# xinjuezou-whi/Open_Duck_Playground

Measured on AMD Instinct MI355X. Metric: env steps/sec (all envs) open_duck_mini_v2 flat, 4096 envs, 1/2/4/8 GPUs, higher is better.
Workload: dtype f32; 1 GPU; C2: flat_terrain, no imitation, 4096 envs per GPU, episode_length 1000 + auto-reset; envs_per_gpu=4096, total_envs=4096, substeps=10, parallelism=env-shard x1, step_kernel=throughput

## Files before the change

### open_duck_playground_amd/csrc/duck_lspairs.h

```cpp
#pragma once
#include "duck_math.h"

typedef float f2v __attribute__((ext_vector_type(2)));

DK float ls_flag_select(float x) { return x < 0.0f ? 1.0f : 0.0f; }
DK float ls_flag_sat(float x) { return __builtin_amdgcn_fmed3f(x * -0x1p127f, 0.0f, 1.0f); }
template <bool SAT>
DK float ls_flag(float x) {
  return SAT ? ls_flag_sat(x) : ls_flag_select(x);
}

template <class Md>
constexpr bool ls_pairs() {
#ifdef DUCK_SCALAR_TWINS
  return false;
#else
  return !(Md::FLOOR_TYPE == 1 && Md::NLIM <= 16);
#endif
}
```

### open_duck_playground_amd/csrc/duck_team.h

```cpp
#pragma once
#include <utility>

#include "duck_ldlpairs.h"
#include "duck_lspairs.h"
#include "duck_mcols.h"
#include "duck_physics.h"

constexpr int TEAM = 16;
constexpr int TEAM_WG = 16;
constexpr int TPB = TEAM * TEAM_WG;
typedef __attribute__((address_space(3))) int lds_int;
typedef float f4v __attribute__((ext_vector_type(4)));
typedef __attribute__((address_space(3))) f4v lds_f4;

DK float frcp(float x) { return __builtin_amdgcn_rcpf(x); }
DK float vsel(unsigned long long m, float t, float f) {
  float r;
  asm("v_cndmask_b32_e64 %0, %1, %2, %3" : "=v"(r) : "v"(f), "v"(t), "s"(m));
  return r;
}

DK float imp_of(const float* solimp, float pos) {
  const float dmin = fminf(fmaxf(solimp[0], 0.0001f), 0.9999f), dmax = fminf(fmaxf(solimp[1], 0.0001f), 0.9999f);
  const float width = fmaxf(1e-15f, solimp[2]), mid = fminf(fmaxf(solimp[3], 0.0001f), 0.9999f);
// ... 2293 lines not shown
      for (int q = 0; q < 3; q++) L[FB + 3 * f + q] = -t[q];
    }
    TSYNC();
    auto sep_of = [&](const float* u) {
      float mx1 = -1e30f, mn2 = 1e30f;
#pragma unroll
      for (int k = 0; k < NH; k++) {
        mx1 = fmaxf(mx1, dot3(u, V1[k]));
        mn2 = fminf(mn2, dot3(u, V2[k]));
      }
      return mn2 - mx1;
    };
    constexpr int NONE = 1 << 20;
    constexpr float TIE = Md::HULL_SAT_TIE;
    constexpr int NFL = (2 * NF + TEAM - 1) / TEAM;
    float fs[NFL], fmx = -1e30f, anysep = 0.0f;
#pragma unroll
    for (int k = 0; k < NFL; k++) {
      const int a = lane + TEAM * k;
      fs[k] = -1e30f;
      if (a < 2 * NF) {
        const int o = a < NF ? FA + 3 * a : FB + 3 * (a - NF);
        const float u[3] = {L[o], L[o + 1], L[o + 2]};
        const float sp = sep_of(u);
        anysep += sp > 0.0f ? 1.0f : 0.0f;
        fs[k] = sp;
      }
      fmx = fmaxf(fmx, fs[k]);
    }
    if (tsum(anysep) > 0.0f) return;
    const float ftop = tmaxf(fmx);
    int mine = NONE;
#pragma unroll
    for (int k = NFL - 1; k >= 0; k--)
      if (fs[k] >= ftop - TIE) mine = lane + TEAM * k;
    const int fbest = tmini(mine);
    float myf = fs[0];
#pragma unroll
    for (int k = 1; k < NFL; k++) myf = fbest / TEAM == k ? fs[k] : myf;
    float best = __shfl(myf, fbest % TEAM, TEAM);
    int btype = fbest / NF, bi = fbest - btype * NF, bj = 0;
    float u_best[3];
    {
      const int o = btype == 0 ? FA + 3 * bi : FB + 3 * bi;
      for (int q = 0; q < 3; q++) u_best[q] = L[o + q];
    }
    constexpr int NEL = (NE + TEAM - 1) / TEAM;
    float EBr[NEL][3], Cr[NEL][3], Dr[NEL][3], DxC[NEL][3];
#pragma unroll
    for (int k = 0; k < NEL; k++) {
      const int e2 = lane + TEAM * k, e2c = e2 < NE ? e2 : 0;
      const int fc = HEF[e2c][0], fd = HEF[e2c][1];
      for (int q = 0; q < 3; q++) {
        EBr[k][q] = L[EB + 3 * e2c + q];
        Cr[k][q] = L[FB + 3 * fc + q];
        Dr[k][q] = L[FB + 3 * fd + q];
      }
      cross3(DxC[k], Dr[k], Cr[k]);
    }
    float esep = -1e30f, eu[3] = {0.0f, 0.0f, 1.0f};
    int eidx = NONE;
    for (int e1 = 0; e1 < NE; e1++) {
      const float ea[3] = {L[EA + 3 * e1], L[EA + 3 * e1 + 1], L[EA + 3 * e1 + 2]};
      const int fa = HEF[e1][0], fb = HEF[e1][1];
      const float A[3] = {L[FA + 3 * fa], L[FA + 3 * fa + 1], L[FA + 3 * fa + 2]};
      const float B[3] = {L[FA + 3 * fb], L[FA + 3 * fb + 1], L[FA + 3 * fb + 2]};
      float BxA[3];
      cross3(BxA, B, A);
      float sepq = 0.0f;
#pragma unroll
      for (int k = 0; k < NEL; k++) {
        const int e2 = lane + TEAM * k;
        const float CBA = dot3(Cr[k], BxA), DBA = dot3(Dr[k], BxA), ADC = dot3(A, DxC[k]), BDC = dot3(B, DxC[k]);
        if (e2 < NE && CBA * DBA < 0.0f && ADC * BDC < 0.0f && CBA * BDC > 0.0f) {
          float u[3];
          cross3(u, ea, EBr[k]);
          const float un = sqrtf(dot3(u, u));
          if (!(un < 1e-6f * sqrtf(dot3(ea, ea)) * sqrtf(dot3(EBr[k], EBr[k])))) {
            u[0] /= un; u[1] /= un; u[2] /= un;
            if (dot3(u, cc) < 0.0f) { u[0] = -u[0]; u[1] = -u[1]; u[2] = -u[2]; }
            const float sp = sep_of(u);
            sepq += sp > 0.0f ? 1.0f : 0.0f;
            if (sp > esep) { esep = sp; eidx = e1 * NE + e2; eu[0] = u[0]; eu[1] = u[1]; eu[2] = u[2]; }
          }
        }
      }
      if (tsum(sepq) > 0.0f) return;
    }
    const float em = tmaxf(esep);
    const int ebest = tmini(esep == em ? eidx : NONE);
    float u_edge[3];
    for (int q = 0; q < 3; q++) u_edge[q] = __shfl(eu[q], (ebest % NE) % TEAM, TEAM);
    if (ebest < NONE && em > best + TIE) {
      best = em;
      btype = 2;
      bi = ebest / NE;
      bj = ebest - bi * NE;
      for (int q = 0; q < 3; q++) u_best[q] = u_edge[q];
    }
    TSYNC();
    float fr[9];
    make_frame(fr, u_best);
    if (btype == 2) {
      float a0[3], a1[3], b0[3], b1[3];
      pick3<NH>(V1, HE[bi][0], a0);
      pick3<NH>(V1, HE[bi][1], a1);
      pick3<NH>(V2, HE[bj][0], b0);
      pick3<NH>(V2, HE[bj][1], b1);
      float d1[3], d2[3], r[3];
      for (int a = 0; a < 3; a++) { d1[a] = a1[a] - a0[a]; d2[a] = b1[a] - b0[a]; r[a] = a0[a] - b0[a]; }
      const float A = dot3(d1, d1), E = dot3(d2, d2), F = dot3(d2, r), C = dot3(d1, r), B = dot3(d1, d2);
      const float den = A * E - B * B;
      float sc = den > 1e-15f ? (B * F - C * E) / den : 0.0f;
      sc = fminf(fmaxf(sc, 0.0f), 1.0f);
      float tt = E > 1e-15f ? (B * sc + F) / E : 0.0f;
      if (tt < 0.0f) { tt = 0.0f; sc = A > 1e-15f ? -C / A : 0.0f; }
      else if (tt > 1.0f) { tt = 1.0f; sc = A > 1e-15f ? (B - C) / A : 0.0f; }
      sc = fminf(fmaxf(sc, 0.0f), 1.0f);
      float pos[3];
      for (int a = 0; a < 3; a++) pos[a] = 0.5f * (a0[a] + sc * d1[a] + b0[a] + tt * d2[a]);
      if (lane == 0) Ph::store_contact(L, slot0, best, pos, fr);
      return;
    }
    const bool ref1 = btype == 0;
    const float* Rr = ref1 ? R1 : R2;
    const float* Ri = ref1 ? R2 : R1;
    const float* pr = ref1 ? p1 : p2;
    float fn[3];
    mulmv3(fn, Rr, HN[bi]);
    const float off = Md::hull_face_offset_d()[bi] + dot3(fn, pr);
    int finc = 0;
    float dmin = 1e30f;
    for (int f = 0; f < NF; f++) {
      float ni[3];
      mulmv3(ni, Ri, HN[f]);
      const float dd = dot3(ni, fn);
      finc = dd < dmin ? f : finc;
      dmin = fminf(dmin, dd);
    }
    constexpr int MFV = Md::HULL_MAXFV, CLIPMAX = 2 * MFV;
    constexpr int PA = EA, PB = EA + 3 * CLIPMAX;
    static_assert(PB + 3 * CLIPMAX <= FA, "clip scratch must fit in the edge storage");
    const int(*FV)[MFV] = Md::hull_face_vert_d();
    const int* FNV = Md::hull_face_nv_d();
    auto vtx = [&](bool h1, int k, float* out) {
      float o1[3], o2[3];
      pick3<NH>(V1, k, o1);
      pick3<NH>(V2, k, o2);
      for (int q = 0; q < 3; q++) out[q] = h1 ? o1[q] : o2[q];
    };
    int np = FNV[finc];
    for (int i = 0; i < np; i++) {
      float v[3];
      vtx(!ref1, FV[finc][i], v);
      for (int q = 0; q < 3; q++) L[PA + 3 * i + q] = v[q];
    }
    int src = PA, dst = PB;
    const int nr = FNV[bi];
    for (int i = 0; i < nr && np > 0; i++) {
      float a[3], b[3], ab[3], sd[3];
      vtx(ref1, FV[bi][i], a);
      vtx(ref1, FV[bi][i + 1 < nr ? i + 1 : 0], b);
      for (int q = 0; q < 3; q++) ab[q] = b[q] - a[q];
      cross3(sd, ab, fn);
      int nt = 0;
      for (int j = 0; j < np; j++) {
        const int jn = j + 1 < np ? j + 1 : 0;
        const float P[3] = {L[src + 3 * j], L[src + 3 * j + 1], L[src + 3 * j + 2]};
        const float Q[3] = {L[src + 3 * jn], L[src + 3 * jn + 1], L[src + 3 * jn + 2]};
        const float dp = sd[0] * (P[0] - a[0]) + sd[1] * (P[1] - a[1]) + sd[2] * (P[2] - a[2]);
        const float dq = sd[0] * (Q[0] - a[0]) + sd[1] * (Q[1] - a[1]) + sd[2] * (Q[2] - a[2]);
        if (dp <= 0.0f && nt < CLIPMAX) {
          for (int q = 0; q < 3; q++) L[dst + 3 * nt + q] = P[q];
          nt++;
        }
        if ((dp <= 0.0f) != (dq <= 0.0f) && nt < CLIPMAX) {
          const float tt = dp / (dp - dq);
          for (int q = 0; q < 3; q++) L[dst + 3 * nt + q] = P[q] + tt * (Q[q] - P[q]);
          nt++;
        }
      }
      TSYNC();
      np = nt;
      const int sw = src;
      src = dst;
      dst = sw;
    }
    float poly[CLIPMAX][3], depth[CLIPMAX];
    bool mask[CLIPMAX], any = false;
#pragma unroll
    for (int k = 0; k < CLIPMAX; k++) {
      const bool ok = k < np;
      for (int q = 0; q < 3; q++) poly[k][q] = ok ? L[src + 3 * k + q] : 0.0f;
      depth[k] = off - dot3(fn, poly[k]);
      mask[k] = ok && depth[k] > 0.0f;
      any = any || mask[k];
    }
    if (!any) return;
    int idx[4];
    manifold_points<CLIPMAX>(poly, mask, fn, idx);
    if (lane < 4) {
      const int c = lane;
      bool unique = true;
      for (int e = 0; e < 4; e++) unique = unique && !(e < c && idx[e] == idx[c]);
      const float dist = unique ? -pick1<CLIPMAX>(depth, idx[c]) : 1.0f;
      float v[3], pos[3];
      pick3<CLIPMAX>(poly, idx[c], v);
      for (int a = 0; a < 3; a++) pos[a] = v[a] - 0.5f * dist * fn[a];
      Ph::store_contact(L, slot0 + c, dist, pos, fr);
    }
  }

  static DNI void collide_hulls_rare(LP L, int lane) {
    constexpr int p = Md::FOOT_PAIR < 0 ? 0 : Md::FOOT_PAIR;
    const int s1 = cgeom_slot<Md>(Md::pair_geom1[p]), s2 = cgeom_slot<Md>(Md::pair_geom2[p]);
    float p1[3], R1[9], p2[3], R2[9], t[3], c1[3], c2[3];
    Ph::geom_frame(L, s1, p1, R1);
    Ph::geom_frame(L, s2, p2, R2);
    const float hc[3] = {Md::hull_center[0], Md::hull_center[1], Md::hull_center[2]};
    mulmv3(t, R1, hc);
    for (int a = 0; a < 3; a++) c1[a] = p1[a] + t[a];
    mulmv3(t, R2, hc);
    for (int a = 0; a < 3; a++) c2[a] = p2[a] + t[a];
    const float cc[3] = {c2[0] - c1[0], c2[1] - c1[1], c2[2] - c1[2]};
    collide_hulls_team(L, lane, 4 * p, p1, R1, p2, R2, cc);
  }

  static DK void collision(LP L, int lane, const float* hf, const ColPre& P) {
    STAGE_T0();
    if constexpr (Md::FLOOR_TYPE == 1) collide_hfield(L, lane, hf);
    else collide_planes(L, lane, P);
    STAGE_MARK(ST_COLLISION_FLOOR);
    if (Md::FOOT_PAIR >= 0) {
      constexpr int p = Md::FOOT_PAIR;
      const int s1 = cgeom_slot<Md>(Md::pair_geom1[p]), s2 = cgeom_slot<Md>(Md::pair_geom2[p]);
      float p1[3], R1[9], p2[3], R2[9], t[3];
      Ph::geom_frame(L, s1, p1, R1);
      Ph::geom_frame(L, s2, p2, R2);
      float c1[3], c2[3];
      const float hc[3] = {Md::hull_center[0], Md::hull_center[1], Md::hull_center[2]};
      mulmv3(t, R1, hc);
      for (int a = 0; a < 3; a++) c1[a] = p1[a] + t[a];
      mulmv3(t, R2, hc);
      for (int a = 0; a < 3; a++) c2[a] = p2[a] + t[a];
      const float cc[3] = {c2[0] - c1[0], c2[1] - c1[1], c2[2] - c1[2]};
      if (dot3(cc, cc) > 4.0f * Md::hull_radius * Md::hull_radius || boxes_separated(p1, R1, p2, R2)) {
        if (lane < 4) {
          const float nofr[9] = {0, 0, 1, 0, 1, 0, -1, 0, 0};
          const float zero[3] = {L[Ly::COM], L[Ly::COM + 1], L[Ly::COM + 2]};
          Ph::store_contact(L, 4 * p + lane, 1.0f, zero, nofr);
        }
      } else {
        TSYNC();
        STAGE_COUNT_IF(lane == 0, ST_N_FOOT_SAT, 1ull);
        collide_hulls_rare(L, lane);
      }
    }
    TSYNC();
  }

  static DK void make_rows(LP L, int lane) {
    if (lane < NFRIC) {
      const int r = lane, i = fric_dof(r);
      L[Ly::RD + r] = tf(Md::B_FRIC + 3 * r + 1);
      L[Ly::AREF + r] = -tf(Md::B_FRIC + 3 * r + 2) * L[Ly::QVEL + i];
    }
    team_for<NLIM>(lane, [&](int r) {
      const int o = Md::B_LIM + LIMW * r;
      const int i = lim_dof(r), qa = lim_qadr(r);
      const float q = L[Ly::QPOS + qa];
      const float dlo = q - tf(o + 2), dhi = tf(o + 3) - q;
      const float pos = fminf(dlo, dhi) - tf(o + 4);
      const float sgn = dlo < dhi ? 1.0f : -1.0f;
      const float k = tf(o + 5), b = tf(o + 6);
      const float si[5] = {tf(o + 8), tf(o + 9), tf(o + 10), tf(o + 11), tf(o + 12)};
      const float imp = imp_of(si, pos);
      const float R = fmaxf(tf(o + 7) * (1.0f - imp) * frcp(imp), 1e-15f);
      const bool active = pos < 0.0f;
      L[Ly::RD + R_LIM + r] = active ? frcp(R) : 0.0f;
      L[Ly::AREF + R_LIM + r] = active ? (-b * sgn * L[Ly::QVEL + i] - k * imp * pos) : 0.0f;
      L[Ly::LSGN + r] = sgn;
    });
    if (lane < NCON) {
      const int slot = lane, p = slot >> 2, o = Md::B_PAIR + PAIRW * p;
      float SL[6], SR[6];
      for (int k = 0; k < 6; k++) { SL[k] = L[Ly::CVEL + 6 * Md::LFOOT_BODY + k]; SR[k] = L[Ly::CVEL + 6 * Md::RFOOT_BODY + k]; }
      const float pos = L[Ly::CDIST + slot] - tf(o + 4);
      const bool active = pos < 0.0f;
      const float k = tf(o + 5), b = tf(o + 6);
      const float si[5] = {tf(o + 8), tf(o + 9), tf(o + 10), tf(o + 11), tf(o + 12)};
      const float imp = imp_of(si, pos);
      const float R = fmaxf(tf(o + 3) * (1.0f - imp) * frcp(imp), 1e-15f);
      float vel[4];
      contact_jx(L, p, slot, SL, SR, vel);
      for (int e = 0; e < 4; e++) {
        const int row = R_CON + 4 * slot + e;
        L[Ly::RD + row] = active ? frcp(R) : 0.0f;
        L[Ly::AREF + row] = active ? (-b * vel[e] - k * imp * pos) : 0.0f;
      }
    }
    TSYNC();
  }

  struct JxIn {
    int s1, s2;
    float mu, r[3], fr[9];
  };
  static DK JxIn jx_load(LP L, int p, int slot) {
    const int o = Md::B_PAIR + PAIRW * p;
    JxIn J;
    J.s1 = ti(o); J.s2 = ti(o + 1); J.mu = tf(o + 2);
    for (int k = 0; k < 3; k++) J.r[k] = L[Ly::CR + Ly::CRS * slot + k];
    for (int k = 0; k < 9; k++) J.fr[k] = L[Ly::CFR + Ly::CFS * slot + k];
    return J;
  }
  static DK void contact_jx(LP L, int p, int slot, const float* SL, const float* SR, float* out4) {
    contact_jx(jx_load(L, p, slot), SL, SR, out4);
  }
  static DK void contact_jx(const JxIn& J, const float* SL, const float* SR, float* out4) {
#pragma clang fp contract(on)
    const int s1 = J.s1, s2 = J.s2;
    const float mu = J.mu;
    const float r[3] = {J.r[0], J.r[1], J.r[2]};
    float v[3] = {0.0f, 0.0f, 0.0f}, t[3];
    if (s2 != 0) { Ph::contact_vel(s2 == 1 ? SL : SR, r, t); v[0] += t[0]; v[1] += t[1]; v[2] += t[2]; }
    if (s1 != 0) { Ph::contact_vel(s1 == 1 ? SL : SR, r, t); v[0] -= t[0]; v[1] -= t[1]; v[2] -= t[2]; }
    float jr[3];
    for (int q = 0; q < 3; q++)
      jr[q] = J.fr[3 * q] * v[0] + J.fr[3 * q + 1] * v[1] + J.fr[3 * q + 2] * v[2];
    out4[0] = jr[0] + mu * jr[1];
    out4[1] = jr[0] - mu * jr[1];
    out4[2] = jr[0] + mu * jr[2];
    out4[3] = jr[0] - mu * jr[2];
  }

  static DK constexpr int kidx(int q, int k) {
    return q <= k ? (q * 6 - (q * (q - 1)) / 2 + (k - q)) : (k * 6 - (k * (k - 1)) / 2 + (q - k));
  }

  struct Pt { float alpha, q0p, q1, q2, d0, d1; };

  static DK void spatial2(LP L, int lane, int X, int X2, float& so, float& so2) {
    so = 0.0f;
    so2 = 0.0f;
    if (lane < 12) {
      int lo = lane;
      asm volatile("" : "+v"(lo));
      const bool left = lo < 6;
      const int k = left ? lo : lo - 6;
      float cvs[Md::MAXCHAIN], xs[Md::MAXCHAIN], x2s[Md::MAXCHAIN];
#pragma unroll
      for (int c = 0; c < Md::MAXCHAIN; c++) {
        const int iL = Md::chain[Md::LFOOT_BODY][c], iR = Md::chain[Md::RFOOT_BODY][c];
        cvs[c] = xs[c] = x2s[c] = 0.0f;
        if (iL < 0 && iR < 0) continue;
        const bool unit = FREE0 && iL == iR && iL >= 0 && iL < 3;
        const int ic = unit ? iL : (left ? (iL >= 0 ? iL : 0) : (iR >= 0 ? iR : 0));
        if (!unit) cvs[c] = L[Ly::CDOF + 6 * ic + k];
        xs[c] = L[X + ic];
        if (X2 >= 0) x2s[c] = L[X2 + ic];
      }
      float s = 0.0f, s2 = 0.0f;
#pragma unroll
      for (int c = 0; c < Md::MAXCHAIN; c++) {
        const int iL = Md::chain[Md::LFOOT_BODY][c], iR = Md::chain[Md::RFOOT_BODY][c];
        if (iL < 0 && iR < 0) continue;
        const bool ok = left ? iL >= 0 : iR >= 0;
        if (FREE0 && iL == iR && iL >= 0 && iL < 3) {
          s += k == 3 + iL ? xs[c] : 0.0f;
          if (X2 >= 0) s2 += k == 3 + iL ? x2s[c] : 0.0f;
          continue;
        }
        const float cd = ok ? cvs[c] : 0.0f;
        s += cd * xs[c];
        if (X2 >= 0) s2 += cd * x2s[c];
      }
      so = s;
      so2 = s2;
    }
  }

  static DK void sp_bcast(float v, float* SL, float* SR) {
    SL[0] = bc<0>(v); SL[1] = bc<1>(v); SL[2] = bc<2>(v); SL[3] = bc<3>(v); SL[4] = bc<4>(v); SL[5] = bc<5>(v);
    SR[0] = bc<6>(v); SR[1] = bc<7>(v); SR[2] = bc<8>(v); SR[3] = bc<9>(v); SR[4] = bc<10>(v); SR[5] = bc<11>(v);
  }

  static DK float fric_cost(float D, float x, float f) {
    const float rf = f * frcp(D);
    const float lo = -f * x - 0.5f * rf * f, hi = f * x - 0.5f * rf * f, qd = 0.5f * D * x * x;
    const float r = x >= rf ? hi : qd;
    return x <= -rf ? lo : r;
  }

  static constexpr int NLR = (NLIM + TEAM - 1) / TEAM;
  struct Rows2 {
    float fja, fv, frf, flin0, ffja, ffv, fQ0, fQ1, fQ2;
    float ja[NLR + 4], v[NLR + 4], Q0[NLR + 4], Q1[NLR + 4], Q2[NLR + 4];
  };
  static DK void set_fric(Rows2& R, float D, float ja, float v, float f) {
    const float rf = f * frcp(D);
    R.fja = ja; R.fv = v; R.frf = rf;
    R.flin0 = -0.5f * rf * f; R.ffja = f * ja; R.ffv = f * v;
    R.fQ0 = 0.5f * D * ja * ja; R.fQ1 = D * v * ja; R.fQ2 = 0.5f * D * v * v;
  }
  static DK void set_row(Rows2& R, int k, float D, float ja, float v) {
    R.ja[k] = ja; R.v[k] = v;
    R.Q0[k] = 0.5f * D * ja * ja; R.Q1[k] = D * v * ja; R.Q2[k] = 0.5f * D * v * v;
  }

  static DK void quad2(const Rows2& R, float alpha, float& q0, float& q1, float& q2) {
    {
      const float x = R.fja + alpha * R.fv;
      const bool lo = x <= -R.frf, hi = x >= R.frf, quad = !(lo || hi);
      const float sg = lo ? -1.0f : 1.0f;
      q0 += quad ? R.fQ0 : R.flin0 + sg * R.ffja;
      q1 += quad ? R.fQ1 : sg * R.ffv;
      q2 += quad ? R.fQ2 : 0.0f;
    }
#pragma unroll
    for (int k = 0; k < NLR + 4; k++) {
      const float on = ls_flag<LS_SAT>(R.ja[k] + alpha * R.v[k]);
      q0 = fmaf(on, R.Q0[k], q0);
      q1 = fmaf(on, R.Q1[k], q1);
      q2 = fmaf(on, R.Q2[k], q2);
    }
  }

  static constexpr bool LS_SAT = ls_pairs<Md>(), LS_PAIRS = LAT == 0 && ls_pairs<Md>();
  static DK void quad2_pair(Rows2& R, f2v alpha, f2v& q0, f2v& q1, f2v& q2) {
    asm("" : "+v"(R.fja), "+v"(R.fv));
#pragma unroll
    for (int k = 0; k < NLR + 4; k++)
      asm("" : "+v"(R.ja[k]), "+v"(R.v[k]), "+v"(R.Q0[k]), "+v"(R.Q1[k]), "+v"(R.Q2[k]));
    {
      const f2v ja = {R.fja, R.fja}, v = {R.fv, R.fv};
      const f2v x = __builtin_elementwise_fma(alpha, v, ja);
      float t0[2], t1[2], t2[2];
#pragma unroll
      for (int h = 0; h < 2; h++) {
        const float xh = h ? x.y : x.x;
        const bool lo = xh <= -R.frf, hi = xh >= R.frf, quad = !(lo || hi);
        const float sg = lo ? -1.0f : 1.0f;
        t0[h] = quad ? R.fQ0 : R.flin0 + sg * R.ffja;
        t1[h] = quad ? R.fQ1 : sg * R.ffv;
        t2[h] = quad ? R.fQ2 : 0.0f;
      }
      q0 += f2v{t0[0], t0[1]};
      q1 += f2v{t1[0], t1[1]};
      q2 += f2v{t2[0], t2[1]};
    }
#pragma unroll
    for (int k = 0; k < NLR + 4; k++) {
      const f2v ja = {R.ja[k], R.ja[k]}, v = {R.v[k], R.v[k]};
      const f2v x = __builtin_elementwise_fma(alpha, v, ja);
      const f2v on = {ls_flag<LS_SAT>(x.x), ls_flag<LS_SAT>(x.y)};
      q0 = __builtin_elementwise_fma(on, f2v{R.Q0[k], R.Q0[k]}, q0);
      q1 = __builtin_elementwise_fma(on, f2v{R.Q1[k], R.Q1[k]}, q1);
      q2 = __builtin_elementwise_fma(on, f2v{R.Q2[k], R.Q2[k]}, q2);
    }
  }

  static DK void solve(LP L, int lane, const float (*Mc)[NV]) {
    STAGE_T0();
    const float g0 = warm_start(L, lane, Mc);
    STAGE_AGAIN(21, (void)warm_start(L, lane, Mc));
    newton(L, lane, Mc, g0);
  }
  struct RowIn { float D, f, sg, ar, w, q; };
  struct DofIn { float fsm, w, q; };
  template <bool W, bool S>
  struct WarmLive {
    LP L;
    int lane, slot;
    DK WarmLive(LP L, int lane) : L(L), lane(lane), slot(lane < NCON ? lane : 0) {}
    DK RowIn fric() const {
      const int r = lane < NFRIC ? lane : 0, i = fric_dof(r);
      return {L[Ly::RD + r], L[Ly::DFRIC + i], 1.0f, L[Ly::AREF + r], W ? L[Ly::WARM + i] : 0.0f,
              S ? L[Ly::QSM + i] : 0.0f};
    }
    DK RowIn lim(int m) const {
      const int rl = lane + TEAM * m, r = rl < NLIM ? rl : 0, i = lim_dof(r);
      return {L[Ly::RD + R_LIM + r], 0.0f, L[Ly::LSGN + r], L[Ly::AREF + R_LIM + r], W ? L[Ly::WARM + i] : 0.0f,
              S ? L[Ly::QSM + i] : 0.0f};
    }
    DK JxIn jx() const { return jx_load(L, slot >> 2, slot); }
    DK RowIn con(int e) const {
      return {L[Ly::RD + R_CON + 4 * slot + e], 0.0f, 1.0f, L[Ly::AREF + R_CON + 4 * slot + e], 0.0f, 0.0f};
    }
    DK DofIn dof(int s) const {
      const int c = TEAM * s + lane, i = c < NV ? c : 0;
      return {L[Ly::FSM + i], L[Ly::WARM + i], L[Ly::QSM + i]};
    }
  };
  struct WarmPre {
    RowIn f, l[NLR], c[4];
    JxIn j;
    DofIn d[NC];
    DK WarmPre(const WarmLive<true, true>& in) {
      f = in.fric();
#pragma unroll
      for (int m = 0; m < NLR; m++) l[m] = in.lim(m);
      j = in.jx();
      for (int e = 0; e < 4; e++) c[e] = in.con(e);
#pragma unroll
      for (int s = 0; s < NC; s++) d[s] = in.dof(s);
    }
    DK RowIn fric() const { return f; }
    DK RowIn lim(int m) const { return l[m]; }
    DK const JxIn& jx() const { return j; }
    DK RowIn con(int e) const { return c[e]; }
    DK DofIn dof(int s) const { return d[s]; }
  };
  static DK float side_cost(float D, float jx) {
    return jx < 0.0f ? 0.5f * D * jx * jx : 0.0f;
  }
  template <bool W, bool S, class V>
  static DK void warm_rows(LP L, int lane, const V& in, const float* SL, const float* SR, const float* SL2,
                           const float* SR2, float& cwp, float& csp) {
    cwp = csp = 0.0f;
    {
      const bool fr = lane < NFRIC;
      const int r = fr ? lane : 0;
      const RowIn x = in.fric();
      const float jw = x.w - x.ar, js = x.q - x.ar;
      if constexpr (W) cwp += fr ? fric_cost(x.D, jw, x.f) : 0.0f;
      if constexpr (S) csp += fr ? fric_cost(x.D, js, x.f) : 0.0f;
      if constexpr (W) L[fr ? Ly::JA + r : TL::SINK + lane] = jw;
      if constexpr (S) L[fr ? Ly::JV + r : TL::SINK + TEAM + lane] = js;
    }
#pragma unroll
    for (int m = 0; m < NLR; m++) {
      const int r = lane + TEAM * m;
      if (NLIM % TEAM != 0 && m == NLR - 1 && r >= NLIM) continue;
      const RowIn x = in.lim(m);
      const float jw = x.sg * x.w - x.ar, js = x.sg * x.q - x.ar;
      if constexpr (W) cwp += side_cost(x.D, jw);
      if constexpr (S) csp += side_cost(x.D, js);
      if constexpr (W) L[Ly::JA + R_LIM + r] = jw;
      if constexpr (S) L[Ly::JV + R_LIM + r] = js;
    }
    if (lane < NCON) {
      const JxIn& jx = in.jx();
      float vw[4] = {}, vs[4] = {};
      if constexpr (W) contact_jx(jx, SL, SR, vw);
      if constexpr (S) contact_jx(jx, SL2, SR2, vs);
      for (int e = 0; e < 4; e++) {
        const int row = R_CON + 4 * lane + e;
        const RowIn x = in.con(e);
        const float jw = vw[e] - x.ar, js = vs[e] - x.ar;
        if constexpr (W) cwp += side_cost(x.D, jw);
        if constexpr (S) csp += side_cost(x.D, js);
        if constexpr (W) L[Ly::JA + row] = jw;
        if constexpr (S) L[Ly::JV + row] = js;
      }
    }
  }
  template <class V>
  static DK float warm_choose(LP L, int lane, const V& in, float cwp, float csp, bool& warm) {
    float gwp = 0.0f;
#pragma unroll
    for (int s = 0; s < NC; s++) {
      const int i = TEAM * s + lane;
      if (NV % TEAM != 0 && s == NC - 1 && i >= NV) continue;
      const DofIn d = in.dof(s);
      gwp += 0.5f * (L[Ly::MA + i] - d.fsm) * (d.w - d.q);
    }
    const float gw = tsum(gwp);
    const float cw = gw + tsum(cwp), cs = tsum(csp);
    float g0;
    warm = cw < cs;
    if (warm) {
      team_for<NV>(lane, [&](int i) { L[Ly::QACC + i] = L[Ly::WARM + i]; });
      g0 = gw;
    } else {
      team_for<NV>(lane, [&](int i) { L[Ly::QACC + i] = L[Ly::QSM + i]; L[Ly::MA + i] = L[Ly::FSM + i]; });
      team_for<NROW>(lane, [&](int r) { L[Ly::JA + r] = L[Ly::JV + r]; });
      g0 = 0.0f;
    }
    TSYNC();
    return g0;
  }
  static DK void warm_start_a0(LP L, int lane, const float (*Mc)[NV], float* SL, float* SR) {
    float sw, ss;
    spatial2(L, lane, Ly::WARM, -1, sw, ss);
    {
      float xw[NC];
      lane_vec(L, lane, Ly::WARM, xw);
      mul_cols(L, lane, Mc, xw, Ly::MA);
    }
    sp_bcast(sw, SL, SR);
  }
  static DK void warm_start_a1(LP L, int lane, const float* SL, const float* SR, float& cwp) {
    float csp;
    warm_rows<true, false>(L, lane, WarmLive<true, false>(L, lane), SL, SR, nullptr, nullptr, cwp, csp);
  }
  static DK float warm_start_b(LP L, int lane, float cwp, bool& warm) {
    float ss, s2;
    spatial2(L, lane, Ly::QSM, -1, ss, s2);
    TSYNC();
    float SL2[6], SR2[6], cw0, csp;
    sp_bcast(ss, SL2, SR2);
    const WarmLive<false, true> in(L, lane);
    warm_rows<false, true>(L, lane, in, nullptr, nullptr, SL2, SR2, cw0, csp);
    return warm_choose(L, lane, in, cwp, csp, warm);
  }
  static DK float warm_start(LP L, int lane, const float (*Mc)[NV]) {
    STAGE_T0();
    const WarmPre P(WarmLive<true, true>(L, lane));
    float sw, ss;
    spatial2(L, lane, Ly::WARM, Ly::QSM, sw, ss);
    {
      float xw[NC];
      lane_vec(L, lane, Ly::WARM, xw);
      mul_cols(L, lane, Mc, xw, Ly::MA);
    }
    TSYNC();
    float SL[6], SR[6], SL2[6], SR2[6], cwp, csp;
    sp_bcast(sw, SL, SR);
    sp_bcast(ss, SL2, SR2);
    STAGE_MARK(ST_WARM_PRODUCTS);
    warm_rows<true, true>(L, lane, P, SL, SR, SL2, SR2, cwp, csp);
    bool warm;
    const float g0 = warm_choose(L, lane, P, cwp, csp, warm);
    STAGE_MARK(ST_WARM_SELECT);
    return g0;
  }
  static DK void newton(LP L, int lane, const float (*Mc)[NV], float g0, bool pre_dir = false) {
    STAGE_T0();
    for (int newton_it = 0;;) {
      bool sparse_ok;
      if (LAT && newton_it == 0 && __ballot(!pre_dir) == 0ull) {
        team_for<NV>(lane, [&](int i) { L[Ly::SRCH + i] = L[TL::XDIR + i]; });
        TSYNC();
        sparse_ok = true;
      } else {
        sparse_ok = newton_fused<false>(L, lane, Mc);
        STAGE_AGAIN(22, sparse_ok = newton_fused<false>(L, lane, Mc));
      }
      STAGE_MARK(ST_NEWTON_DIR);
      if (sparse_ok) {
        STAGE_MARK(ST_NEWTON_SPARSE);
      } else {
        TSYNC();
        STAGE_COUNT_IF(lane == 0, ST_N_DENSE_FALLBACK, 1ull);
        newton_dense(L, lane);
        TSYNC();
      }
      struct SearchPre {
        float fD, fja, ff, lD[NLR], lja[NLR], lsg[NLR], cD[4], cja[4], ma[NC], fsm[NC];
        JxIn jx;
      } SP;
      {
        const int slot = lane < NCON ? lane : 0;
        SP.jx = jx_load(L, slot >> 2, slot);
        const int r = lane < NFRIC ? lane : 0;
        SP.fD = L[Ly::RD + r]; SP.fja = L[Ly::JA + r]; SP.ff = L[Ly::DFRIC + fric_dof(r)];
#pragma unroll
        for (int m = 0; m < NLR; m++) {
          const int rl = lane + TEAM * m, rc = rl < NLIM ? rl : 0;
          SP.lD[m] = L[Ly::RD + R_LIM + rc]; SP.lja[m] = L[Ly::JA + R_LIM + rc]; SP.lsg[m] = L[Ly::LSGN + rc];
        }
        for (int e = 0; e < 4; e++) {
          SP.cD[e] = L[Ly::RD + R_CON + 4 * slot + e]; SP.cja[e] = L[Ly::JA + R_CON + 4 * slot + e];
        }
#pragma unroll
        for (int s = 0; s < NC; s++) {
          const int c = TEAM * s + lane, cc = c < NV ? c : 0;
          SP.ma[s] = L[Ly::MA + cc]; SP.fsm[s] = L[Ly::FSM + cc];
        }
      }
      float sv, sv2;
      spatial2(L, lane, Ly::SRCH, -1, sv, sv2);
      {
        float xs[NC];
        lane_vec(L, lane, Ly::SRCH, xs);
        mul_cols(L, lane, Mc, xs, Ly::GRAD);
      }
      TSYNC();
      Rows2 R;
      {
        const bool fr = lane < NFRIC;
        const int r = fr ? lane : 0, i = fric_dof(r);
        const float D = SP.fD, ja = SP.fja, v = L[Ly::SRCH + i], f = SP.ff;
        set_fric(R, fr ? D : 1.0f, fr ? ja : 0.0f, fr ? v : 0.0f, fr ? f : 0.0f);
      }
#pragma unroll
      for (int m = 0; m < NLR; m++) {
        const int r = lane + TEAM * m;
        const bool ok = r < NLIM;
        const int rc = ok ? r : 0, i = lim_dof(rc);
        const float D = SP.lD[m], ja = SP.lja[m], v = SP.lsg[m] * L[Ly::SRCH + i];
        set_row(R, m, ok ? D : 0.0f, ok ? ja : 0.0f, ok ? v : 0.0f);
      }
      {
        float SL[6], SR[6], v[4];
        sp_bcast(sv, SL, SR);
        contact_jx(SP.jx, SL, SR, v);
        for (int e = 0; e < 4; e++) {
          const bool ok = lane < NCON;
          const float D = SP.cD[e], ja = SP.cja[e];
          set_row(R, NLR + e, ok ? D : 0.0f, ok ? ja : 0.0f, ok ? v[e] : 0.0f);
        }
      }
      float sn = 0.0f, sMa = 0.0f, sf = 0.0f, sMv = 0.0f;
      LS_DUMP_START(L, lane);
#pragma unroll
      for (int s = 0; s < NC; s++) {
        const int i = TEAM * s + lane;
        if (NV % TEAM != 0 && s == NC - 1 && i >= NV) continue;
        const float sv = L[Ly::SRCH + i];
        sn += sv * sv;
        sMa += sv * SP.ma[s];
        sf += sv * SP.fsm[s];
        sMv += sv * L[Ly::GRAD + i];
      }
      LS_DUMP_NORM(L, lane, sn);
      sn = tsum(sn); sMa = tsum(sMa); sf = tsum(sf); sMv = tsum(sMv);
      STAGE_MARK(ST_SEARCH_PRODUCTS);
      const float gtol = Md::tolerance * Md::ls_tolerance * sqrtf(sn) * Md::meaninertia * (float)(NV > 1 ? NV : 1);
      const float G0 = g0, G1 = sMa - sf, G2 = 0.5f * sMv;
      auto mk = [&](float alpha, float q0, float q1, float q2) {
        q1 = tsum(q1) + G1; q2 = tsum(q2) + G2;
        Pt p;
        p.alpha = alpha;
        p.q0p = q0;
        p.q1 = q1;
        p.q2 = q2;
        p.d0 = 2.0f * alpha * q2 + q1;
        p.d1 = 2.0f * q2;
        return p;
      };
      auto cost = [&](const Pt& p) { return p.alpha * p.alpha * p.q2 + p.alpha * p.q1 + (tsum(p.q0p) + G0); };
      Pt p0;
      {
        float q0 = 0, q1 = 0, q2 = 0;
        quad2(R, 0.0f, q0, q1, q2);
        LS_DUMP_QUAD(L, lane, q0, q1, q2, G0, G1, G2, gtol, sn);
        p0 = mk(0.0f, q0, q1, q2);
      }
      Pt lo;
      {
        const float a1 = p0.alpha - p0.d0 * frcp(p0.d1);
        float q0 = 0, q1 = 0, q2 = 0;
        quad2(R, a1, q0, q1, q2);
        lo = mk(a1, q0, q1, q2);
      }
      Pt hi;
      if (lo.d0 < p0.d0) { hi = p0; } else { hi = lo; lo = p0; }
      bool swap = true;
      const float gtol_ls = fmaxf(gtol, LS_SLOPE_FLOOR * fabsf(p0.d0));
      STAGE_PROF_ONLY(int its = 0;)
      for (int it = 0; it < Md::ls_iterations; it++) {
        bool done = !swap;
        done = done || ((lo.d0 < 0.0f) && (lo.d0 > -gtol_ls));
        done = done || ((hi.d0 > 0.0f) && (hi.d0 < gtol_ls));
        if (done) break;
        STAGE_PROF_ONLY(its = it + 1;)
        STAGE_COUNT_WAVE0(ST_N_LS_WAVE_ITERS, 1ull);
        const float al = lo.alpha - lo.d0 / lo.d1, ah = hi.alpha - hi.d0 / hi.d1, am = 0.5f * (lo.alpha + hi.alpha);
        float a0 = 0, a1 = 0, a2 = 0, b0 = 0, b1 = 0, b2 = 0, c0 = 0, c1 = 0, c2 = 0;
        if constexpr (LS_PAIRS) {
          f2v p0 = {0.0f, 0.0f}, p1 = {0.0f, 0.0f}, p2 = {0.0f, 0.0f};
          quad2_pair(R, f2v{al, ah}, p0, p1, p2);
          a0 = p0.x; b0 = p0.y; a1 = p1.x; b1 = p1.y; a2 = p2.x; b2 = p2.y;
        } else {
          quad2(R, al, a0, a1, a2);
          quad2(R, ah, b0, b1, b2);
        }
        quad2(R, am, c0, c1, c2);
        const Pt lo_next = mk(al, a0, a1, a2), hi_next = mk(ah, b0, b1, b2), mid = mk(am, c0, c1, c2);
        const bool s1 = (lo.d0 > 0.0f) || (lo.d0 < lo_next.d0);
        if (s1) lo = lo_next;
        const bool s2 = (mid.d0 < 0.0f) && (lo.d0 < mid.d0);
        if (s2) lo = mid;
        const bool s3 = (hi.d0 < 0.0f) || (hi.d0 > hi_next.d0);
        if (s3) hi = hi_next;
        const bool s4 = (mid.d0 > 0.0f) && (hi.d0 > mid.d0);
        if (s4) hi = mid;
        swap = s1 || s2 || s3 || s4;
      }
      STAGE_PROF_ONLY(if (threadIdx.x < 64 && (lane & 15) == 0) {
        STAGE_COUNT(ST_N_LS_TEAM_ITERS, (unsigned long long)its);
        STAGE_COUNT(ST_N_LS_SEARCHES, 1ull);
      })
      const float lo_cost = cost(lo), hi_cost = cost(hi), p0_cost = cost(p0);
      const bool improved = (lo_cost < p0_cost) || (hi_cost < p0_cost);
      const float alpha = lo_cost < hi_cost ? lo.alpha : hi.alpha;
      if (improved)
        team_for<NV>(lane, [&](int i) { L[Ly::QACC + i] += L[Ly::SRCH + i] * alpha; });
      TSYNC();
      STAGE_MARK(ST_LINESEARCH);
      if constexpr (Md::iterations <= 1) {
        break;
      } else {
        if (++newton_it >= Md::iterations) break;
        const float a = improved ? alpha : 0.0f;
        const float cnew = improved ? (lo_cost < hi_cost ? lo_cost : hi_cost) : p0_cost;
        g0 = G0 + a * G1 + a * a * G2;
        team_for<NV>(lane, [&](int i) { L[Ly::MA + i] += a * L[Ly::GRAD + i]; });
        if (lane < NFRIC) L[Ly::JA + lane] = R.fja + a * R.fv;
#pragma unroll
        for (int m = 0; m < NLR; m++) {
          const int r = lane + TEAM * m;
          if (r < NLIM) L[Ly::JA + R_LIM + r] = R.ja[m] + a * R.v[m];
        }
        if (lane < NCON)
          for (int e = 0; e < 4; e++) L[Ly::JA + R_CON + 4 * lane + e] = R.ja[NLR + e] + a * R.v[NLR + e];
        TSYNC();
        const float scale = 1.0f / (Md::meaninertia * (float)(NV > 1 ? NV : 1));
        if (scale * (p0_cost - cnew) < Md::tolerance) break;
      }
    }
  }

  static DK void sensors(LP L, int lane) {
    const float com[3] = {L[Ly::COM], L[Ly::COM + 1], L[Ly::COM + 2]};
    float cacc1[6];
    for (int k = 0; k < 6; k++) cacc1[k] = (k >= 3) ? -Md::gravity[k - 3] : 0.0f;
    for (int i = 0; i < 6; i++) {
      const float v = L[Ly::QVEL + i], a = L[Ly::QACC + i];
      for (int k = 0; k < 6; k++) {
        const float cdd = i >= 3 ? L[Ly::CDD1 + 6 * (i - 3) + k] : 0.0f;
        cacc1[k] += cdd * v + L[Ly::CDOF + 6 * i + k] * a;
      }
    }
    for (int s = lane; s < Md::NSENSOR; s += TEAM) {
      const int os = Md::B_SENS + 20 * s;
      const int typ = ti(os), site = ti(os + 1), adr = ti(os + 2), b = ti(os + 3);
      float R[9], sp[3], sR[9], t[3], SM[9];
      const float spos[3] = {tf(os + 4), tf(os + 5), tf(os + 6)};
      for (int k = 0; k < 9; k++) { R[k] = L[Ly::XMAT + Ly::XMS * b + k]; SM[k] = tf(os + 7 + k); }
      mulmv3(t, R, spos);
      for (int k = 0; k < 3; k++) sp[k] = L[Ly::XPOS + Ly::XPS * b + k] + t[k];
      mulmm3(sR, R, SM);
      const float off[3] = {sp[0] - com[0], sp[1] - com[1], sp[2] - com[2]};
      float ang[3] = {L[Ly::CVEL + 6 * b], L[Ly::CVEL + 6 * b + 1], L[Ly::CVEL + 6 * b + 2]}, lin[3];
      cross3(t, ang, off);
      for (int k = 0; k < 3; k++) lin[k] = L[Ly::CVEL + 6 * b + 3 + k] + t[k];
      float o[4] = {0.0f, 0.0f, 0.0f, 0.0f};
      if (typ == 0) mulmtv3(o, sR, ang);
      else if (typ == 1) mulmtv3(o, sR, lin);
      else if (typ == 2) {
        float acc[3];
        cross3(t, cacc1, off);
        for (int k = 0; k < 3; k++) acc[k] = cacc1[3 + k] + t[k];
        cross3(t, ang, lin);
        for (int k = 0; k < 3; k++) acc[k] += t[k];
        mulmtv3(o, sR, acc);
      } else if (typ == 3) { o[0] = sR[2]; o[1] = sR[5]; o[2] = sR[8]; }
      else if (typ == 4) { o[0] = sR[0]; o[1] = sR[3]; o[2] = sR[6]; }
      else if (typ == 5) { o[0] = lin[0]; o[1] = lin[1]; o[2] = lin[2]; }
      else if (typ == 6) { o[0] = ang[0]; o[1] = ang[1]; o[2] = ang[2]; }
      else if (typ == 7) { o[0] = sp[0]; o[1] = sp[1]; o[2] = sp[2]; }
      else if (typ == 8) {
        const float bq[4] = {L[Ly::XQ + 4 * b], L[Ly::XQ + 4 * b + 1], L[Ly::XQ + 4 * b + 2], L[Ly::XQ + 4 * b + 3]};
        const float sq[4] = {tf(os + 16), tf(os + 17), tf(os + 18), tf(os + 19)};
        qmul(o, bq, sq);
        qnormalize(o);
      }
      const int dim = typ == 8 ? 4 : 3;
      for (int k = 0; k < dim; k++) L[Ly::SENS + adr + k] = o[k];
      if (typ == 0 && site == Md::IMU_SITE) { L[Ly::IMUR] = sR[6]; L[Ly::IMUR + 1] = sR[7]; L[Ly::IMUR + 2] = sR[8]; }
      if (typ == 7 && site == Md::LFOOT_SITE) L[Ly::FOOTZ] = sp[2];
      if (typ == 7 && site == Md::RFOOT_SITE) L[Ly::FOOTZ + 1] = sp[2];
    }
    {
      constexpr int p0 = Md::PLANE_PAIR[0], p1 = Md::PLANE_PAIR[1];
      constexpr int s20 = cgeom_slot<Md>(Md::pair_geom2[p0]), s21 = cgeom_slot<Md>(Md::pair_geom2[p1]);
      const int p = lane == 0 ? p0 : p1, s2 = lane == 0 ? s20 : s21;
      float mn = 1e4f;
      for (int c = 0; c < 4; c++) mn = fminf(mn, L[Ly::CDIST + 4 * p + c]);
      L[lane < 2 ? Ly::OCON + s2 - 1 : TL::SINK + lane] = mn < 0.0f ? 1.0f : 0.0f;
    }
    TSYNC();
  }

  static DK void euler(LP L, int lane) {
    const float dt = Md::timestep;
    team_all<NV>(lane, [&](int i, bool ok) {
      const float qa = L[Ly::QACC + i], qv = L[Ly::QVEL + i];
      L[ok ? Ly::WARM + i : TL::SINK + lane] = qa;
      L[ok ? Ly::QVEL + i : TL::SINK + TEAM + lane] = qv + dt * qa;
    });
    TSYNC();
    {
      float qp[3];
      for (int k = 0; k < 3; k++) qp[k] = L[Ly::QPOS + k] + dt * L[Ly::QVEL + k];
      const float v[3] = {L[Ly::QVEL + 3], L[Ly::QVEL + 4], L[Ly::QVEL + 5]};
      const float nvv = sqrtf(dot3(v, v));
      float ax[3] = {1.0f, 0.0f, 0.0f};
      if (nvv > 1e-15f) { ax[0] = v[0] / nvv; ax[1] = v[1] / nvv; ax[2] = v[2] / nvv; }
      float s, c;
      __sincosf(0.5f * dt * nvv, &s, &c);
      const float qr[4] = {c, ax[0] * s, ax[1] * s, ax[2] * s};
      float q[4] = {L[Ly::QPOS + 3], L[Ly::QPOS + 4], L[Ly::QPOS + 5], L[Ly::QPOS + 6]};
      qmul(q, q, qr);
      qnormalize(q);
      for (int k = 0; k < 3; k++) L[Ly::QPOS + k] = qp[k];
      for (int k = 0; k < 4; k++) L[Ly::QPOS + 3 + k] = q[k];
    }
    team_for<NJ, 1>(lane, [&](int j) {
      const int oj = Md::B_JREC + 9 * j;
      const bool jh = Md::B_JAFF && j >= Md::B_JN0;
      const int qa = jh ? j + Md::B_JQD : ti(oj + 2), da = jh ? j + Md::B_JDD : ti(oj + 1);
      L[Ly::QPOS + qa] += dt * L[Ly::QVEL + da];
    });
    TSYNC();
  }

  static DK void end_substep(LP L, int lane, bool integrate) {
    if (integrate) {
      euler(L, lane);
    } else {
      team_for<NV>(lane, [&](int i) { L[Ly::WARM + i] = L[Ly::QACC + i]; });
      TSYNC();
    }
  }

  static DK void step(LP L, int lane, bool integrate, bool want_out, float* aux, int aux_stride, const float* hf) {
    STAGE_T0();
    const ComPre cp = com_pre(L, lane);
    kinematics(L, lane);
    STAGE_AGAIN(6, kinematics(L, lane));
    STAGE_MARK(ST_KINEMATICS);
    const RnePre rp = rne_pre(L, lane);
    com_pos(L, lane, cp);
// ... 237 lines not shown
```

Baseline: 22.88 million env-steps/s.

## Keep warm-start row jacobians in registers and pair warm/smooth evaluation

The warm-start stage now evaluates the warm and smooth candidates together in two-wide float vectors. This covers the spatial chain sums, friction, limit and contact rows. The row residuals stay in registers instead of being written to LDS, and the warm-or-smooth choice is applied with predicated stores, which removes the separate JA/JV copy pass. Contact Jacobian velocity is computed branch-free unless a guarded configuration applies. The cost is higher register pressure and some redundant contact_vel work when a side is inactive.

```diff
diff --git a/open_duck_playground_amd/csrc/duck_lspairs.h b/open_duck_playground_amd/csrc/duck_lspairs.h
--- a/open_duck_playground_amd/csrc/duck_lspairs.h
+++ b/open_duck_playground_amd/csrc/duck_lspairs.h
@@ -18,3 +18,12 @@
   return !(Md::FLOOR_TYPE == 1 && Md::NLIM <= 16);
 #endif
 }
+
+template <class Md>
+constexpr bool warm_pairs() {
+#if defined(DUCK_SCALAR_TWINS) || defined(DUCK_SCALAR_WARM)
+  return false;
+#else
+  return true;
+#endif
+}
diff --git a/open_duck_playground_amd/csrc/duck_team.h b/open_duck_playground_amd/csrc/duck_team.h
--- a/open_duck_playground_amd/csrc/duck_team.h
+++ b/open_duck_playground_amd/csrc/duck_team.h
@@ -2619,6 +2619,7 @@
     TSYNC();
   }
 
+  static constexpr bool JX_GUARDED = LAT == 2 && Md::FLOOR_TYPE == 1 && Md::NLIM > 16;
   struct JxIn {
     int s1, s2;
     float mu, r[3], fr[9];
@@ -2639,9 +2640,23 @@
     const int s1 = J.s1, s2 = J.s2;
     const float mu = J.mu;
     const float r[3] = {J.r[0], J.r[1], J.r[2]};
-    float v[3] = {0.0f, 0.0f, 0.0f}, t[3];
-    if (s2 != 0) { Ph::contact_vel(s2 == 1 ? SL : SR, r, t); v[0] += t[0]; v[1] += t[1]; v[2] += t[2]; }
-    if (s1 != 0) { Ph::contact_vel(s1 == 1 ? SL : SR, r, t); v[0] -= t[0]; v[1] -= t[1]; v[2] -= t[2]; }
+    float v[3] = {0.0f, 0.0f, 0.0f};
+    if constexpr (!JX_GUARDED) {
+      float S2[6], S1[6], t2[3], t1[3];
+#pragma unroll
+      for (int k = 0; k < 6; k++) { S2[k] = s2 == 1 ? SL[k] : SR[k]; S1[k] = s1 == 1 ? SL[k] : SR[k]; }
+      Ph::contact_vel(S2, r, t2);
+      Ph::contact_vel(S1, r, t1);
+#pragma unroll
+      for (int a = 0; a < 3; a++) {
+        const float va = s2 != 0 ? t2[a] : 0.0f, vb = va - t1[a];
+        v[a] = s1 != 0 ? vb : va;
+      }
+    } else {
+      float t[3];
+      if (s2 != 0) { Ph::contact_vel(s2 == 1 ? SL : SR, r, t); v[0] += t[0]; v[1] += t[1]; v[2] += t[2]; }
+      if (s1 != 0) { Ph::contact_vel(s1 == 1 ? SL : SR, r, t); v[0] -= t[0]; v[1] -= t[1]; v[2] -= t[2]; }
+    }
     float jr[3];
     for (int q = 0; q < 3; q++)
       jr[q] = J.fr[3 * q] * v[0] + J.fr[3 * q + 1] * v[1] + J.fr[3 * q + 2] * v[2];
@@ -2695,6 +2710,44 @@
       so = s;
       so2 = s2;
     }
+  }
+
+  static DK void spatial2_pair(LP L, int lane, int X, int X2, float& so, float& so2) {
+#pragma clang fp contract(off)
+    f2v s = {0.0f, 0.0f};
+    if (lane < 12) {
+      int lo = lane;
+      asm volatile("" : "+v"(lo));
+      const bool left = lo < 6;
+      const int k = left ? lo : lo - 6;
+      float cvs[Md::MAXCHAIN];
+      f2v xs[Md::MAXCHAIN];
+#pragma unroll
+      for (int c = 0; c < Md::MAXCHAIN; c++) {
+        const int iL = Md::chain[Md::LFOOT_BODY][c], iR = Md::chain[Md::RFOOT_BODY][c];
+        cvs[c] = 0.0f;
+        xs[c] = f2v{0.0f, 0.0f};
+        if (iL < 0 && iR < 0) continue;
+        const bool unit = FREE0 && iL == iR && iL >= 0 && iL < 3;
+        const int ic = unit ? iL : (left ? (iL >= 0 ? iL : 0) : (iR >= 0 ? iR : 0));
+        if (!unit) cvs[c] = L[Ly::CDOF + 6 * ic + k];
+        xs[c] = f2v{L[X + ic], L[X2 + ic]};
+      }
+#pragma unroll
+      for (int c = 0; c < Md::MAXCHAIN; c++) {
+        const int iL = Md::chain[Md::LFOOT_BODY][c], iR = Md::chain[Md::RFOOT_BODY][c];
+        if (iL < 0 && iR < 0) continue;
+        const bool ok = left ? iL >= 0 : iR >= 0;
+        if (FREE0 && iL == iR && iL >= 0 && iL < 3) {
+          const bool on = k == 3 + iL;
+          s += f2v{on ? xs[c].x : 0.0f, on ? xs[c].y : 0.0f};
+          continue;
+        }
+        s = pfma(sp2(ok ? cvs[c] : 0.0f), xs[c], s);
+      }
+    }
+    so = s.x;
+    so2 = s.y;
   }
 
   static DK void sp_bcast(float v, float* SL, float* SR) {
@@ -2872,6 +2925,121 @@
       }
     }
   }
+  struct RowJ { f2v f, l[NLR], c[4]; };
+  template <class V>
+  static DK void warm_rows_both(LP L, int lane, const V& in, const float* SL, const float* SR, const float* SL2,
+                                const float* SR2, float& cwp, float& csp, RowJ& K) {
+    if constexpr (warm_pairs<Md>()) {
+      warm_rows_pair(L, lane, in, SL, SR, SL2, SR2, cwp, csp, K);
+      return;
+    }
+    cwp = csp = 0.0f;
+    {
+      const bool fr = lane < NFRIC;
+      const RowIn x = in.fric();
+      const float jw = x.w - x.ar, js = x.q - x.ar;
+      const float fw = fric_cost(x.D, jw, x.f), fs = fric_cost(x.D, js, x.f);
+      cwp += fr ? fw : 0.0f;
+      csp += fr ? fs : 0.0f;
+      K.f = f2v{jw, js};
+    }
+#pragma unroll
+    for (int m = 0; m < NLR; m++) {
+      const bool ok = TEAM * (m + 1) <= NLIM || lane + TEAM * m < NLIM;
+      const RowIn x = in.lim(m);
+      const float jw = x.sg * x.w - x.ar, js = x.sg * x.q - x.ar;
+      const float lw = side_cost(x.D, jw), ls = side_cost(x.D, js);
+      cwp += ok ? lw : 0.0f;
+      csp += ok ? ls : 0.0f;
+      K.l[m] = f2v{jw, js};
+    }
+    {
+      const bool ok = lane < NCON;
+      const JxIn& jx = in.jx();
+      float vw[4], vs[4];
+      contact_jx(jx, SL, SR, vw);
+      contact_jx(jx, SL2, SR2, vs);
+#pragma unroll
+      for (int e = 0; e < 4; e++) {
+        const RowIn x = in.con(e);
+        const float jw = vw[e] - x.ar, js = vs[e] - x.ar;
+        const float ew = side_cost(x.D, jw), es = side_cost(x.D, js);
+        cwp += ok ? ew : 0.0f;
+        csp += ok ? es : 0.0f;
+        K.c[e] = f2v{jw, js};
+      }
+    }
+  }
+  static DK f2v sp2(float a) { return f2v{a, a}; }
+  static DK f2v pfma(f2v a, f2v b, f2v c) { return __builtin_elementwise_fma(a, b, c); }
+  static DK f2v side_cost2(float D, f2v j, bool ok) {
+#pragma clang fp contract(off)
+    const f2v q = sp2(0.5f * D) * j * j;
+    return f2v{ok && j.x < 0.0f ? q.x : 0.0f, ok && j.y < 0.0f ? q.y : 0.0f};
+  }
+  template <class V>
+  static DK void warm_rows_pair(LP L, int lane, const V& in, const float* SL, const float* SR, const float* SL2,
+                                const float* SR2, float& cwp, float& csp, RowJ& K) {
+#pragma clang fp contract(off)
+    f2v c;
+    {
+      const bool fr = lane < NFRIC;
+      const RowIn x = in.fric();
+      const f2v j = f2v{x.w, x.q} - sp2(x.ar);
+      const float rf = x.f * frcp(x.D), t = 0.5f * rf * x.f;
+      const f2v lo = pfma(j, sp2(-x.f), sp2(-t)), hi = pfma(sp2(x.f), j, sp2(-t)), qd = sp2(0.5f * x.D) * j * j;
+      const float rw = j.x >= rf ? hi.x : qd.x, rs = j.y >= rf ? hi.y : qd.y;
+      const float fw = j.x <= -rf ? lo.x : rw, fs = j.y <= -rf ? lo.y : rs;
+      c = f2v{fr ? fw : 0.0f, fr ? fs : 0.0f};
+      K.f = j;
+    }
+#pragma unroll
+    for (int m = 0; m < NLR; m++) {
+      const int rl = lane + TEAM * m;
+      const bool ok = TEAM * (m + 1) <= NLIM || rl < NLIM;
+      const RowIn x = in.lim(m);
+      const f2v j = pfma(f2v{x.w, x.q}, sp2(x.sg), sp2(-x.ar));
+      c += side_cost2(x.D, j, ok);
+      K.l[m] = j;
+    }
+    {
+      const bool ok = lane < NCON;
+      const JxIn& J = in.jx();
+      const bool l2 = J.s2 == 1, l1 = J.s1 == 1, n2 = J.s2 != 0, n1 = J.s1 != 0;
+      f2v A[6], B[6];
+#pragma unroll
+      for (int k = 0; k < 6; k++) {
+        A[k] = f2v{l2 ? SL[k] : SR[k], l2 ? SL2[k] : SR2[k]};
+        B[k] = f2v{l1 ? SL[k] : SR[k], l1 ? SL2[k] : SR2[k]};
+      }
+      const f2v r0 = sp2(J.r[0]), r1 = sp2(J.r[1]), r2 = sp2(J.r[2]);
+      const f2v t[3] = {A[3] + pfma(r2, A[1], -(r1 * A[2])), pfma(r0, A[2], -(r2 * A[0])) + A[4],
+                        pfma(r1, A[0], -(r0 * A[1])) + A[5]};
+      const f2v u[3] = {pfma(r1, B[2], -(r2 * B[1])) - B[3], pfma(r2, B[0], -(r0 * B[2])) - B[4],
+                        pfma(r0, B[1], -(r1 * B[0])) - B[5]};
+      f2v v[3];
+#pragma unroll
+      for (int a = 0; a < 3; a++) {
+        const f2v va = {n2 ? t[a].x : 0.0f, n2 ? t[a].y : 0.0f}, vb = va + u[a];
+        v[a] = f2v{n1 ? vb.x : va.x, n1 ? vb.y : va.y};
+      }
+      f2v jr[3];
+#pragma unroll
+      for (int q = 0; q < 3; q++)
+        jr[q] = pfma(sp2(J.fr[3 * q + 2]), v[2], pfma(sp2(J.fr[3 * q]), v[0], sp2(J.fr[3 * q + 1]) * v[1]));
+      const f2v mu = sp2(J.mu);
+      const f2v o4[4] = {pfma(mu, jr[1], jr[0]), pfma(-mu, jr[1], jr[0]), pfma(mu, jr[2], jr[0]),
+                         pfma(-mu, jr[2], jr[0])};
+#pragma unroll
+      for (int e = 0; e < 4; e++) {
+        const RowIn x = in.con(e);
+        K.c[e] = o4[e] - sp2(x.ar);
+        c += side_cost2(x.D, K.c[e], ok);
+      }
+    }
+    cwp = c.x;
+    csp = c.y;
+  }
   template <class V>
   static DK float warm_choose(LP L, int lane, const V& in, float cwp, float csp, bool& warm) {
     float gwp = 0.0f;
@@ -2897,6 +3065,43 @@
     TSYNC();
     return g0;
   }
+  template <class V>
+  static DK float warm_choose_kept(LP L, int lane, const V& in, float cwp, float csp, const RowJ& K) {
+    float gwp = 0.0f, ma[NC];
+#pragma unroll
+    for (int s = 0; s < NC; s++) {
+      const int c = TEAM * s + lane;
+      const bool ok = TEAM * (s + 1) <= NV || c < NV;
+      const DofIn d = in.dof(s);
+      ma[s] = L[Ly::MA + (ok ? c : 0)];
+      const float g = gwp + 0.5f * (ma[s] - d.fsm) * (d.w - d.q);
+      gwp = ok ? g : gwp;
+    }
+    const float gw = tsum(gwp);
+    const float cw = gw + tsum(cwp), cs = tsum(csp);
+    const bool warm = cw < cs;
+#pragma unroll
+    for (int s = 0; s < NC; s++) {
+      const int c = TEAM * s + lane;
+      const bool ok = TEAM * (s + 1) <= NV || c < NV;
+      const DofIn d = in.dof(s);
+      L[ok ? Ly::QACC + c : TL::SINK + lane] = warm ? d.w : d.q;
+      L[ok ? Ly::MA + c : TL::SINK + TEAM + lane] = warm ? ma[s] : d.fsm;
+    }
+    L[lane < NFRIC ? Ly::JA + lane : TL::SINK + lane] = warm ? K.f.x : K.f.y;
+#pragma unroll
+    for (int m = 0; m < NLR; m++) {
+      const int rl = lane + TEAM * m;
+      const bool ok = TEAM * (m + 1) <= NLIM || rl < NLIM;
+      L[ok ? Ly::JA + R_LIM + rl : TL::SINK + lane] = warm ? K.l[m].x : K.l[m].y;
+    }
+    if (lane < NCON) {
+#pragma unroll
+      for (int e = 0; e < 4; e++) L[Ly::JA + R_CON + 4 * lane + e] = warm ? K.c[e].x : K.c[e].y;
+    }
+    TSYNC();
+    return warm ? gw : 0.0f;
+  }
   static DK void warm_start_a0(LP L, int lane, const float (*Mc)[NV], float* SL, float* SR) {
     float sw, ss;
     spatial2(L, lane, Ly::WARM, -1, sw, ss);
@@ -2925,7 +3130,8 @@
     STAGE_T0();
     const WarmPre P(WarmLive<true, true>(L, lane));
     float sw, ss;
-    spatial2(L, lane, Ly::WARM, Ly::QSM, sw, ss);
+    if constexpr (warm_pairs<Md>()) spatial2_pair(L, lane, Ly::WARM, Ly::QSM, sw, ss);
+    else spatial2(L, lane, Ly::WARM, Ly::QSM, sw, ss);
     {
       float xw[NC];
       lane_vec(L, lane, Ly::WARM, xw);
@@ -2936,9 +3142,9 @@
     sp_bcast(sw, SL, SR);
     sp_bcast(ss, SL2, SR2);
     STAGE_MARK(ST_WARM_PRODUCTS);
-    warm_rows<true, true>(L, lane, P, SL, SR, SL2, SR2, cwp, csp);
-    bool warm;
-    const float g0 = warm_choose(L, lane, P, cwp, csp, warm);
+    RowJ K;
+    warm_rows_both(L, lane, P, SL, SR, SL2, SR2, cwp, csp, K);
+    const float g0 = warm_choose_kept(L, lane, P, cwp, csp, K);
     STAGE_MARK(ST_WARM_SELECT);
     return g0;
   }
```

Result: faster. 23.21 million env-steps/s, median of 6 (+1.5%).
